# peterropac/Aegolius

Measured on AMD Instinct MI355X. Metric: Mpoints/sec SDF eval, 1024^3 grid, 10-prim smooth-union tree, higher is better.
Workload: dtype f32

## Files before the change

### aegolius_amd/_engine.py

```python
import atexit
import contextlib
import ctypes
import importlib.util
import os
import sys
import threading

import numpy as np

_HERE = os.path.dirname(os.path.abspath(__file__))
LIB_PATH = os.path.join(_HERE, "libsdfk.so")

MODE_AUTO, MODE_INTERPRET, MODE_SPECIALIZED, MODE_NOCULL = 0, 1, 2, 3
(FLAVOUR_PLAIN_ARRAY, FLAVOUR_PLAIN_GRID, FLAVOUR_TILE_ARRAY, FLAVOUR_TILE_GRID, FLAVOUR_TILE_MASK, FLAVOUR_ROWS_ARRAY,
 FLAVOUR_ROWS_GRID, FLAVOUR_ROWS_MASK, FLAVOUR_ROWS2D_ARRAY, FLAVOUR_ROWS2D_GRID, FLAVOUR_RAYS, FLAVOUR_OCCUPANCY) = range(12)
FLAVOUR_FLAGS = 0x100
FLAVOUR_XY = 0x200

_c = ctypes
_vp, _i64, _int, _sz = _c.c_void_p, _c.c_int64, _c.c_int, _c.c_size_t
_fp = _c.POINTER(_c.c_float)

SIGNATURES = {
    "sdfk_abi_version": (_int, []),
    "sdfk_device_count": (_int, []),
    "sdfk_last_error": (_c.c_char_p, []),
    "sdfk_program_create": (_vp, [_vp, _sz, _vp, _sz, _vp, _sz, _int]),
    "sdfk_program_destroy": (None, [_vp]),
    "sdfk_program_set_params": (_int, [_vp, _vp, _sz]),
    "sdfk_program_set_cull": (_int, [_vp, _vp, _sz, _vp]),
    "sdfk_program_source": (_c.c_char_p, [_vp]),
    "sdfk_program_compile_check": (_int, [_vp, _c.POINTER(_sz)]),
    "sdfk_program_chain_members": (_int, [_vp]),
    "sdfk_program_compile_flavour": (_int, [_vp, _int, _c.POINTER(_sz), _c.POINTER(_c.c_double)]),
    "sdfk_debug_compile_external": (_int, [_vp, _int, _c.POINTER(_sz)]),
    "sdfk_debug_jit_stats": (None, [_c.POINTER(_i64), _c.POINTER(_c.c_double)]),
    "sdfk_jit_drain": (None, []),
    "sdfk_jit_cancel": (None, []),
    "sdfk_debug_set_rtc_defs": (None, [_c.c_char_p]),
    "sdfk_eval_device": (_int, [_vp, _vp, _i64, _i64, _vp, _vp, _int]),
    "sdfk_eval_device_rows": (_int, [_vp, _vp, _i64, _i64, _i64, _vp, _vp, _int]),
    "sdfk_eval_device_rows2d": (_int, [_vp, _vp, _i64, _i64, _i64, _vp, _vp, _int]),
    "sdfk_eval_device_rows2d_xy": (_int, [_vp, _vp, _i64, _i64, _i64, _vp, _vp, _int]),
    "sdfk_debug_cells_stats": (None, [_int, _c.POINTER(_c.c_longlong)]),
    "sdfk_debug_rays_stats": (None, [_int, _c.POINTER(_c.c_longlong)]),
    "sdfk_eval_device_rows3d": (_int, [_vp, _vp, _i64, _i64, _i64, _i64, _i64, _vp, _vp, _int]),
    "sdfk_debug_row_masks": (_int, [_vp, _vp, _i64, _i64, _i64, _vp, _c.POINTER(_i64), _c.POINTER(_int), _vp]),
    "sdfk_eval_grid_sharded": (_int, [_vp, _vp, _i64, _vp, _i64, _vp, _i64, _int, _vp, _vp, _int]),
    "sdfk_eval_grid_sharded_device": (_int, [_vp, _vp, _i64, _vp, _i64, _vp, _i64, _int, _vp, _int, _vp, _int]),
    "sdfk_eval_device_aux": (_int, [_vp, _vp, _i64, _i64, _vp, _int, _i64, _vp, _vp, _int]),
    "sdfk_eval_grid_aux": (_int, [_vp, _vp, _i64, _vp, _i64, _vp, _i64, _i64, _i64, _vp, _int, _i64, _vp, _vp, _int]),
    "sdfk_field_min": (_int, [_vp, _i64, _c.POINTER(_c.c_float), _vp]),
    "sdfk_grid_box_average": (_int, [_vp, _i64, _i64, _i64, _int, _int, _int, _int, _vp, _vp]),
    "sdfk_grid_edge_detect": (_int, [_vp, _i64, _i64, _i64, _vp, _vp]),
# ... 114 lines not shown
        with _lock:
            if _lib is None:
                if not os.path.exists(LIB_PATH):
                    raise SdfkError(
                        "aegolius_amd: %s is missing - build it with "
                        "`python -c 'import __graft_entry__ as g; g.build()'` (needs hipcc, gfx950). "
                        "There is no CPU path." % LIB_PATH)
                _share_torch_hip_runtime()
                handle = ctypes.CDLL(LIB_PATH)
                for name, (res, args) in SIGNATURES.items():
                    fn = getattr(handle, name)
                    fn.restype, fn.argtypes = res, args
                if handle.sdfk_abi_version() != 1:
                    raise SdfkError("libsdfk.so ABI version mismatch")
                atexit.register(handle.sdfk_jit_cancel)
                _lib = handle
    return _lib


def last_error():
    msg = lib().sdfk_last_error()
    return msg.decode("utf-8", "replace") if msg else ""


def check(rc, what):
    if rc != 0:
        raise SdfkError("%s failed (%d): %s" % (what, rc, last_error()))


def device_count():
# ... 581 lines not shown
```

### aegolius_amd/csrc/sdfk.hip

```cpp
#include <hip/hip_runtime.h>
#include <hip/hiprtc.h>

#include <chrono>
#include <algorithm>
#include <atomic>
#include <cmath>
#include <condition_variable>
#include <cstdio>
#include <cstdlib>
#include <cstring>
#include <deque>
#include <functional>
#include <map>
#include <memory>
#include <mutex>
#include <thread>
#include <string>
#include <vector>
#include <dirent.h>
#include <dlfcn.h>
#include <fcntl.h>
#include <signal.h>
#include <spawn.h>
#include <sys/wait.h>
// ... 1053 lines not shown
    if (e->state == 0) {
        e->state = 1;
        lk.unlock();
        const std::string src = make_source();
        if (wait || !rtc_helper_available()) {
            code_build(e, src, rwb);
        } else {
            g_builds.post([e, src, rwb] { code_build(e, src, rwb, true); });
        }
        return e;
    }
    if (wait) e->cv.wait(lk, [&] { return e->state != 1; });
    return e;
}
static std::string flavour_key(const sdfk_program* p, int flavour, int rwb, int with_flags = 0) {
    return p->key + "|f" + std::to_string(flavour) + ((with_flags & 1) ? "s" : "") + ((with_flags & 2) ? "x" : "") + "|" + rtc_option_key(rwb);
}
static std::string flavour_source(const sdfk_program* p, int flavour, int with_flags = 0) {
    return std::string((with_flags & 1) ? "#define SDFK_FLAGS 1\n" : "") + ((with_flags & 2) ? "#define SDFK_XY 1\n" : "") +
           sdfk_generate_source(g_ops, SDFK_OP_COUNT, p->code.data(), p->code.size() / 2, p->result_reg, p->sites, flavour,
                                &p->sites_all);
}

extern "C" int sdfk_program_chain_members(const sdfk_program* p) {
    return p && p->chain_mode ? p->chain_members : 0;
}
extern "C" int sdfk_program_compile_check(sdfk_program* p, size_t* code_size) {
    if (!p) return fail(-1, "null program");
    size_t total = 0;
    const int rwb = rows_geo(p);
    for (int f = 0; f < SDFK_FL_COUNT; ++f) {
        if (f == SDFK_FL_RAYS) continue;
        if (f == SDFK_FL_OCCUPANCY) continue;
        if (p->sites.empty() && f != SDFK_FL_PLAIN_ARRAY && f != SDFK_FL_PLAIN_GRID) continue;
// ... 310 lines not shown
            g_cells_stats[6] = (long long)all; g_cells_stats[7] = (long long)empty;
        }
        if (trace) fprintf(stderr, "[sdfk cells] %d members: fine %ux%ux%u = %llu cells (2^%u planes x 2^%u blocks x 2^%u windows), coarse %llu; pool %u of %llu entries; "
                "fine lists: mean %.1f max %llu, %llu without a list, %llu empty\n", p->chain_members, fine.ncx, fine.ncy, fine.ncz, nf, fine.lx, fine.ly, fine.lz, nc,
                head, cap, (double)sum / (double)std::max<unsigned long long>(1, nf - all - empty), mx, all, empty);
    }
    out->lv = fine;
    out->sph = b + o_fsph;
    out->span = b + o_fspan;
    out->cand = b + o_pool;
    out->enabled = 1u;
    out->ncells = (unsigned)nf;
    return 0;
}

static int run(sdfk_program* p, const SrcArray* arr, const SrcGrid* grid, long long n, float* d_out, void* stream_,
               int mode, bool vec_ok, long long row_len = 0, const float* aux = nullptr, long long aux_stride = 0,
               bool flat = false, long long plane_rows = 0, long long plane_phase = 0, unsigned* d_flags = nullptr,
               unsigned thr_key = 0, bool xy = false) {
    if (!p) return fail(-1, "null program");
    if (n < 0) return fail(-1, "negative point count");
    if (p->n_aux > 0 && (!aux || aux_stride < n))
        return fail(-1, "this program reads auxiliary fields (staged evaluation): use sdfk_eval_device_aux / sdfk_eval_grid_aux");
    if (n == 0) return 0;
    if (mode == SDFK_MODE_AUTO) mode = g_default_mode;
    if (d_flags && (mode == SDFK_MODE_AUTO || mode == SDFK_MODE_INTERPRET)) mode = SDFK_MODE_SPECIALIZED;
    if (xy) {
        if (!arr || p->n_aux > 0) return fail(-1, "two-row coordinates: array source, no auxiliary fields");
        if (mode == SDFK_MODE_AUTO || mode == SDFK_MODE_INTERPRET) mode = SDFK_MODE_SPECIALIZED;
    }
    hipStream_t stream = (hipStream_t)stream_;
    int device = 0;
    HIPCHK(hipGetDevice(&device));
    DevState* d = nullptr;
// ... 23 lines not shown
        if (arr && rows_geometry(n, row_len, &rg, (flat || d_flags) ? 0 : plane_rows, plane_phase, p->chain_mode))
            flavour = (flat || xy) ? SDFK_FL_ROWS2D_ARRAY : SDFK_FL_ROWS_ARRAY;
        else if (arr && vec_ok && !p->chain_mode && !d_flags && !xy) flavour = SDFK_FL_TILE_ARRAY;
        else if (grid && grid->start % grow == 0 &&
                 rows_geometry(n, grow, &rg, (grid->n2 > 1 && !d_flags) ? (long long)grid->n1 : 0,
                               grid->n2 > 1 ? (grid->start / grow) % (long long)grid->n1 : 0, p->chain_mode))
            flavour = grid->n2 > 1 ? SDFK_FL_ROWS_GRID : SDFK_FL_ROWS2D_GRID;
        else if (grid && vec_ok && !p->chain_mode && !d_flags) flavour = SDFK_FL_TILE_GRID;
        if (!p->chain_mode && (long long)(p->code.size() / 2) > rows_limit &&
            (flavour == SDFK_FL_ROWS_ARRAY || flavour == SDFK_FL_ROWS2D_ARRAY || flavour == SDFK_FL_ROWS_GRID || flavour == SDFK_FL_ROWS2D_GRID)) {
            const bool is_arr = arr != nullptr;
            if (vec_ok && !d_flags && !xy) flavour = is_arr ? SDFK_FL_TILE_ARRAY : SDFK_FL_TILE_GRID;
            else if (!d_flags) flavour = is_arr ? SDFK_FL_PLAIN_ARRAY : SDFK_FL_PLAIN_GRID;
        }
    }
    std::shared_ptr<SpecModule> sk;
    if (mode != SDFK_MODE_INTERPRET) {
        static const bool async_jit = [] { const char* e = getenv("SDFK_ASYNC_JIT"); return !(e && e[0] == '0'); }();
        const bool wait = mode != SDFK_MODE_AUTO || !p->interp_ok || !async_jit;
        std::string err;
        sk = get_module(p, device, flavour, wait, &err, (d_flags ? 1 : 0) | (xy ? 2 : 0));
        if (sk && sk->failed) {
            if (mode == SDFK_MODE_SPECIALIZED || !p->interp_ok)
                return fail(-3, "specialised kernel unavailable: " + err);
            static bool warned = false;
            if (!warned) {
                fprintf(stderr, "[sdfk] hiprtc specialisation failed, using the interpreter kernel: %s\n", err.c_str());
                warned = true;
            }
            sk.reset();
        }
    }
    if (!sk && !p->interp_ok)
        return fail(-4, "program needs more registers than the interpreter kernel has (use the specialised mode)");

    const float* prm = d->d_params;
// ... 13 lines not shown
                    void* src[] = {&co, &stride};
                    rc = prepare_cells(p, d, sk->fn[1], rg, src, 2, prm, tab, stream, &cells);
                    if (rc) return rc;
                }
                void* args[] = {&prm, &tab, &co, &stride, &rg, &d_out, &d_flags, &thr_key, &cells};
                HIPCHK(hipModuleLaunchKernel(sk->fn[0], tiles, 1, 1, rthreads, 1, 1, 0, stream, args, nullptr));
            } else {
                SrcGrid g = *grid;
                rg.row0 = grid->start / grow;
                rg.yrows = grid->n2 > 1 ? 0 : 1;
                if (with_cells) {
                    void* src[] = {&g};
                    rc = prepare_cells(p, d, sk->fn[1], rg, src, 1, prm, tab, stream, &cells);
                    if (rc) return rc;
                }
                void* args[] = {&prm, &tab, &g, &rg, &d_out, &d_flags, &thr_key, &cells};
                HIPCHK(hipModuleLaunchKernel(sk->fn[0], tiles, 1, 1, rthreads, 1, 1, 0, stream, args, nullptr));
            }
            return 0;
        }
        if (flavour == SDFK_FL_TILE_ARRAY || flavour == SDFK_FL_TILE_GRID) {
            const unsigned tiles = (unsigned)((n + tile_points() - 1) / tile_points());
            if (arr) {
                const float* co = arr->co;
                long long stride = arr->stride;
                void* args[] = {&prm, &tab, &co, &stride, &n, &d_out};
                HIPCHK(hipModuleLaunchKernel(sk->fn[0], tiles, 1, 1, tile_threads(), 1, 1, 0, stream, args, nullptr));
            } else {
                SrcGrid g = *grid;
                void* args[] = {&prm, &tab, &g, &n, &d_out};
                HIPCHK(hipModuleLaunchKernel(sk->fn[0], tiles, 1, 1, tile_threads(), 1, 1, 0, stream, args, nullptr));
// ... 188 lines not shown
    if (n == 1) {
        out[0] = (float)lo;
        return 0;
    }
    const double div = (double)(n - 1);
    const double delta = hi - lo;
    const double step = delta / div;
    for (int64_t i = 0; i < n; ++i) {
        volatile double t = (step != 0.0) ? (double)i * step : ((double)i / div) * delta;
        out[i] = (float)(t + lo);
    }
    out[n - 1] = (float)hi;
    return 0;
}

struct AxisTables {
    float* d = nullptr;
    ~AxisTables() {
        if (d) (void)hipFree(d);
    }
};

static int upload_axes(const float* ax0, int64_t n0, const float* ax1, int64_t n1, const float* ax2, int64_t n2,
                       hipStream_t stream, AxisTables* t, SrcGrid* g, int64_t start) {
    if (!ax0 || !ax1 || !ax2 || n0 < 1 || n1 < 1 || n2 < 1) return fail(-1, "grid axes missing or empty");
    if (n1 > 0x7fffffff || n2 > 0x7fffffff) return fail(-1, "grid axis too long");
    HIPCHK(hipMalloc(&t->d, (size_t)(n0 + n1 + n2) * sizeof(float)));
    HIPCHK(hipMemcpyAsync(t->d, ax0, (size_t)n0 * sizeof(float), hipMemcpyHostToDevice, stream));
    HIPCHK(hipMemcpyAsync(t->d + n0, ax1, (size_t)n1 * sizeof(float), hipMemcpyHostToDevice, stream));
    HIPCHK(hipMemcpyAsync(t->d + n0 + n1, ax2, (size_t)n2 * sizeof(float), hipMemcpyHostToDevice, stream));
    g->ax0 = t->d;
    g->ax1 = t->d + n0;
    g->ax2 = t->d + n0 + n1;
    g->n1 = (unsigned)n1;
    g->n2 = (unsigned)n2;
    g->start = start;
    return 0;
}

extern "C" int sdfk_eval_grid(sdfk_program* p, const float* ax0, int64_t n0, const float* ax1, int64_t n1,
                              const float* ax2, int64_t n2, int64_t start, int64_t count, float* d_out, void* stream,
                              int mode) {
    if (!d_out) return fail(-1, "sdfk_eval_grid: null output");
    if (start < 0 || count < 0 || start + count > n0 * n1 * n2) return fail(-1, "sdfk_eval_grid: range outside the grid");
    AxisTables t;
    SrcGrid g;
    int rc = upload_axes(ax0, n0, ax1, n1, ax2, n2, (hipStream_t)stream, &t, &g, start);
    if (rc) return rc;
    rc = run(p, nullptr, &g, count, d_out, stream, mode, aligned16(d_out));
    if (rc) return rc;
    HIPCHK(hipStreamSynchronize((hipStream_t)stream));
    return 0;
}

extern "C" int sdfk_eval_grid_aux(sdfk_program* p, const float* ax0, int64_t n0, const float* ax1, int64_t n1,
                                  const float* ax2, int64_t n2, int64_t start, int64_t count, const float* d_aux, int n_aux,
                                  int64_t aux_stride, float* d_out, void* stream, int mode) {
    if (!p || !d_out) return fail(-1, "sdfk_eval_grid_aux: null pointer");
    if (start < 0 || count < 0 || start + count > n0 * n1 * n2) return fail(-1, "sdfk_eval_grid_aux: range outside the grid");
    if (n_aux < p->n_aux) return fail(-1, "sdfk_eval_grid_aux: the program reads more auxiliary fields than were passed");
    AxisTables t;
    SrcGrid g;
    int rc = upload_axes(ax0, n0, ax1, n1, ax2, n2, (hipStream_t)stream, &t, &g, start);
    if (rc) return rc;
    rc = run(p, nullptr, &g, count, d_out, stream, mode, aligned16(d_out), 0, d_aux, aux_stride);
    if (rc) return rc;
    HIPCHK(hipStreamSynchronize((hipStream_t)stream));
    return 0;
}

extern "C" int sdfk_eval_grid_host(sdfk_program* p, const float* ax0, int64_t n0, const float* ax1, int64_t n1,
                                   const float* ax2, int64_t n2, int64_t start, int64_t count, float* out, int device,
                                   int mode) {
    if (!p) return fail(-1, "null program");
    if (count < 0 || (count > 0 && !out)) return fail(-1, "sdfk_eval_grid_host: bad arguments");
    if (start < 0 || start + count > n0 * n1 * n2) return fail(-1, "sdfk_eval_grid_host: range outside the grid");
    if (count == 0) return 0;
    HIPCHK(hipSetDevice(device));
    int64_t chunk = std::min<int64_t>(count, (int64_t)1 << 27);
    const int64_t grow = n2 > 1 ? n2 : n1;
    if (start % grow == 0 && chunk > grow) chunk = chunk / grow * grow;
    float* d_out = nullptr;
    HIPCHK(hipMalloc(&d_out, (size_t)chunk * sizeof(float)));
    AxisTables t;
    SrcGrid g;
    int rc = upload_axes(ax0, n0, ax1, n1, ax2, n2, nullptr, &t, &g, start);
    for (int64_t s = 0; s < count && rc == 0; s += chunk) {
        const int64_t m = std::min(chunk, count - s);
        g.start = start + s;
        rc = run(p, nullptr, &g, m, d_out, nullptr, mode, true);
        if (rc == 0 && hipMemcpy(out + s, d_out, (size_t)m * sizeof(float), hipMemcpyDeviceToHost) != hipSuccess)
            rc = fail(-6, "sdfk_eval_grid_host: device-to-host copy failed");
    }
    (void)hipFree(d_out);
    return rc;
}

extern "C" int sdfk_eval_grid_sharded(sdfk_program* p, const float* ax0, int64_t n0, const float* ax1, int64_t n1,
                                      const float* ax2, int64_t n2, int n_shards, const int* devices, float* out,
                                      int mode) {
    if (!p || !out) return fail(-1, "sdfk_eval_grid_sharded: null argument");
    if (n_shards < 1 || n_shards > 64) return fail(-1, "sdfk_eval_grid_sharded: 1..64 shards");
    if (!ax0 || !ax1 || !ax2 || n0 < 1 || n1 < 1 || n2 < 1) return fail(-1, "grid axes missing or empty");
    int n_dev = 0;
    if (hipGetDeviceCount(&n_dev) != hipSuccess || n_dev < 1) return fail(-8, "sdfk_eval_grid_sharded: no HIP device");
// ... 367 lines not shown
```

### aegolius_amd/csrc/sdfk_codegen.cpp

```cpp
#include "sdfk_codegen.h"

#include <algorithm>
#include <cstdio>
#include <cstring>
#include <map>
#include <set>

#include "sdfk_embedded.inc"

std::string sdfk_vector_prelude() { return std::string(kEmbeddedDevice) + "\n" + kEmbeddedVecdev + "\n"; }

static const char kWrappers[] = R"SDFKW(
template <int VEC, typename SRC>
static __device__ __forceinline__ void sdfk_body(const float* __restrict__ PRM, const float* __restrict__ TAB,
                                                 const SRC& src, long long off, long long n,
                                                 float* __restrict__ out, const float* __restrict__ aux,
                                                 long long aux_stride, unsigned* __restrict__ flags, unsigned thr) {
    const long long block_base = (long long)sdfk_bx() * (SDFK_BLOCK * VEC);
    const unsigned lane_off = sdfk_tx() * VEC;
#ifdef SDFK_FLAGS                                              // the flag-writing build of this flavour (its own code object:
    {                                                          // carried as a run-time branch it cost the field kernels registers)
        const bool active = block_base + lane_off < n;
        unsigned nib = 0u;
        if (active) {
// ... 1678 lines not shown
static const char kRowsGrid[] = R"SDFKR(
// the same on a regular grid expanded from three per-axis tables (no coordinate array: 4 B/point); the slab
// starts at a row boundary and out[0] is its first point
extern "C" __global__ __launch_bounds__(64 * SDFK_RWAVES) void sdfk_spec_rg(
    const float* __restrict__ PRM, const float* __restrict__ TAB, SrcGrid s, sdfk_rowgeom g, float* __restrict__ out,
    unsigned* __restrict__ flags, unsigned thr SDFK_CELLS_KARG) {
    sdfk_rows_kernel(PRM, TAB, s, g, out, flags, thr SDFK_CELLS_PASS);
}
#ifdef SDFK_CELLS
extern "C" __global__ __launch_bounds__(256) void sdfk_spec_cellsg(
    const float* __restrict__ PRM, const float* __restrict__ TAB, SrcGrid s, sdfk_rowgeom g, sdfk_cellpass cp) {
    sdfk_cells_kernel(PRM, TAB, s, g, cp);
}
#endif
)SDFKR";
static const char kRowsMask[] = R"SDFKR(
// test aid: the skip masks (two 64-bit words per brick: sites 0-31, 32-63; bit 2k = first operand of site k
// skipped, bit 2k+1 = second) followed by the "uniform rows" flag in a third word
extern "C" __global__ __launch_bounds__(64 * SDFK_RWAVES) void sdfk_spec_rmask(
    const float* __restrict__ PRM, const float* __restrict__ TAB, const float* __restrict__ co, long long stride,
    sdfk_rowgeom g, unsigned long long* __restrict__ masks) {
    __shared__ __attribute__((aligned(16))) sdfk_rowmeta meta;
    const SrcArray s = {co, stride};
    unsigned rb, c;
    sdfk_rows_prepare(PRM, TAB, s, g, &meta, sdfk_bx(), rb, c);
    const unsigned q = sdfk_bx() * SDFK_RNBRICK + sdfk_tx();
    if (sdfk_tx() < SDFK_RNBRICK && q < g.nbricks) {
        masks[3ull * q] = meta.mask[0][sdfk_tx()];
        masks[3ull * q + 1] = meta.mask[1][sdfk_tx()];
        masks[3ull * q + 2] = meta.uniform[sdfk_tx()];
// ... 980 lines not shown
               "    return x;\n}\n";
        g.simt = g.analyse_leaves();
        if (g.simt) {
            char def[160];
            snprintf(def, sizeof def, "\n#ifndef SDFK_NOSIMT\n#define SDFK_SIMT 1\n#endif\n#define SDFK_NLEAF %zu\n", g.leaves.size());
            g.s += def;
            g.s += kSimtGeometry;
            g.emit_groups();
            g.emit_probe_leaves();
            g.emit_probe_fold();
        }
        g.emit_probe();
        g.emit_rows_culled(result_reg);
        g.s += kRowsKernel;
        if (all || flavour == SDFK_FL_ROWS_ARRAY || flavour == SDFK_FL_ROWS2D_ARRAY) g.s += kRowsArray;
        if (all || flavour == SDFK_FL_ROWS_GRID || flavour == SDFK_FL_ROWS2D_GRID) g.s += kRowsGrid;
        if (all || flavour == SDFK_FL_ROWS_MASK) g.s += kRowsMask;
    }
    return g.s;
}
```

### aegolius_amd/csrc/sdfk_occupancy.inc

```
#include "sdfk_occdev.h"

template <int NC, int NV, typename SRC>
__global__ __launch_bounds__(SDFK_OCC_BLOCK) void sdfk_occ_interp_kernel(const uint2* __restrict__ code, int n_instr,
                                                                        const float* __restrict__ prm,
                                                                        const float* __restrict__ tab, int result_reg, SRC src,
                                                                        sdfk_occgrid grid, float* __restrict__ out) {
    const SdfkInterpField<NC, NV> field = {code, n_instr, prm, tab, result_reg};
    sdfk_occ_sample(src, field, grid, out);
}

#define SDFK_OCC_RUN 1024
#define SDFK_OCC_PARTIALS 4096

struct sdfk_occclass {
    const float* __restrict__ ax0;
    const float* __restrict__ ax1;
    const float* __restrict__ ax2;
    const float* __restrict__ hw0;
    const float* __restrict__ hw1;
    const float* __restrict__ hw2;
    unsigned n1, n2;
    long long first, count;
    float level, lip;
    unsigned level_key;
// ... 173 lines not shown
    const unsigned k0 = n0 > 1 ? samples : 1, k1 = n1 > 1 ? samples : 1, k2 = n2 > 1 ? samples : 1;
    auto lg = [](unsigned k) { return k == 8 ? 3u : k == 4 ? 2u : k == 2 ? 1u : 0u; };
    const unsigned K = k0 * k1 * k2;
    const int64_t total_cells = n0 * n1 * n2;
    const int64_t slab = occ_slab_cells(n0, n1, n2, slab_cells);

    hipStream_t stream = (hipStream_t)stream_;
    int device = 0;
    HIPCHK(hipGetDevice(&device));
    DevState* d = nullptr;
    int rc = ensure_resident(p, device, stream, &d);
    if (rc) return rc;

    AxisTables axes, extra;
    SrcGrid g;
    rc = upload_axes(ax0, n0, ax1, n1, ax2, n2, stream, &axes, &g, 0);
    if (rc) return rc;
    const size_t s0 = (size_t)n0 * k0, s1 = (size_t)n1 * k1, s2 = (size_t)n2 * k2;
    HIPCHK(hipMalloc(&extra.d, (s0 + s1 + s2 + (size_t)(n0 + n1 + n2)) * sizeof(float)));
    float* d_sub[3] = {extra.d, extra.d + s0, extra.d + s0 + s1};
    float* d_hw[3] = {extra.d + s0 + s1 + s2, extra.d + s0 + s1 + s2 + n0, extra.d + s0 + s1 + s2 + n0 + n1};
    HIPCHK(hipMemcpyAsync(d_sub[0], sub0, s0 * sizeof(float), hipMemcpyHostToDevice, stream));
    HIPCHK(hipMemcpyAsync(d_sub[1], sub1, s1 * sizeof(float), hipMemcpyHostToDevice, stream));
    HIPCHK(hipMemcpyAsync(d_sub[2], sub2, s2 * sizeof(float), hipMemcpyHostToDevice, stream));
    HIPCHK(hipMemcpyAsync(d_hw[0], hw0, (size_t)n0 * sizeof(float), hipMemcpyHostToDevice, stream));
    HIPCHK(hipMemcpyAsync(d_hw[1], hw1, (size_t)n1 * sizeof(float), hipMemcpyHostToDevice, stream));
    HIPCHK(hipMemcpyAsync(d_hw[2], hw2, (size_t)n2 * sizeof(float), hipMemcpyHostToDevice, stream));

    char* scratch = (char*)d_scratch;
    unsigned long long* d_partial = (unsigned long long*)scratch;
    unsigned long long* d_blk = (unsigned long long*)(scratch + SDFK_OCC_PARTIALS * 8);
// ... 11 lines not shown
    sdfk_occclass C = {g.ax0, g.ax1, g.ax2, d_hw[0], d_hw[1], d_hw[2], (unsigned)n1, (unsigned)n2, 0, 0, level, lipschitz,
                       sdfk_sel_key(level)};
    const float* prm = d->d_params;
    const float* tab = d->d_tables;
    const int n_instr = (int)(p->code.size() / 2);
    const unsigned per_wave = K >= 64u ? 1u : 64u / K;
    int64_t near_total = 0;

    for (int64_t first = 0; first < total_cells; first += slab) {
        const int64_t cells = std::min(slab, total_cells - first);
        float* out = d_fraction + first;
        unsigned long long n_entries = (unsigned long long)cells;
        if (pass_ms) HIPCHK(hipEventRecord(ev.e[0], stream));
        if (skip) {
            g.start = first;
            rc = run(p, nullptr, &g, cells, d_centre, stream, mode, true);
            if (rc) return rc;
            if (pass_ms) HIPCHK(hipEventRecord(ev.e[1], stream));
            C.first = first;
            C.count = cells;
            const long long runs = occ_runs(cells);
            const unsigned blocks = (unsigned)((runs + SDFK_OCC_BLOCK / 64 - 1) / (SDFK_OCC_BLOCK / 64));
            hipLaunchKernelGGL(sdfk_occ_classify_kernel<false>, dim3(blocks), dim3(SDFK_OCC_BLOCK), 0, stream,
                               (const float*)d_centre, C, out, d_list, d_blk);
            hipLaunchKernelGGL(sdfk_select_scan_kernel, dim3(1), dim3(1024), 0, stream, d_blk, runs);
            hipLaunchKernelGGL(sdfk_occ_classify_kernel<true>, dim3(blocks), dim3(SDFK_OCC_BLOCK), 0, stream,
                               (const float*)d_centre, C, out, d_list, d_blk);
            HIPCHK(hipGetLastError());
            unsigned long long h = 0;
            HIPCHK(hipMemcpyAsync(&h, d_blk + runs, sizeof h, hipMemcpyDeviceToHost, stream));
            HIPCHK(hipStreamSynchronize(stream));
// ... 69 lines not shown
```

### include/sdfk.h

```cpp
#ifndef SDFK_H
#define SDFK_H

#include <stddef.h>
#include <stdint.h>

#ifdef __cplusplus
extern "C" {
#endif

#define SDFK_ABI_VERSION 1

#define SDFK_MODE_AUTO 0
#define SDFK_MODE_INTERPRET 1
#define SDFK_MODE_SPECIALIZED 2
#define SDFK_MODE_NOCULL 3

typedef struct sdfk_program sdfk_program;

int sdfk_abi_version(void);
int sdfk_device_count(void);
const char* sdfk_last_error(void);

sdfk_program* sdfk_program_create(const uint32_t* code, size_t n_instr, const float* params, size_t n_params,
                                  const float* tables, size_t n_tables, int result_reg);
// ... 13 lines not shown
#define SDFK_FLAVOUR_ROWS_MASK 7
#define SDFK_FLAVOUR_ROWS2D_ARRAY 8
#define SDFK_FLAVOUR_ROWS2D_GRID 9
#define SDFK_FLAVOUR_RAYS 10
#define SDFK_FLAVOUR_OCCUPANCY 11
#define SDFK_FLAVOUR_FLAGS 0x100
#define SDFK_FLAVOUR_XY 0x200
int sdfk_program_compile_flavour(sdfk_program* prog, int flavour, size_t* code_size, double* seconds);
void sdfk_debug_cells_stats(int enable, long long* out8);
void sdfk_debug_rays_stats(int enable, long long* out8);
int sdfk_debug_compile_external(sdfk_program* prog, int flavour, size_t* code_size);
void sdfk_jit_drain(void);
void sdfk_jit_cancel(void);
void sdfk_debug_jit_stats(int64_t* builds, double* seconds);
void sdfk_debug_set_rtc_defs(const char* defs);

int sdfk_eval_device(sdfk_program* prog, const float* d_co, int64_t n, int64_t row_stride, float* d_out,
                     void* stream, int mode);
int sdfk_eval_device_rows(sdfk_program* prog, const float* d_co, int64_t n, int64_t row_stride, int64_t row_len,
                          float* d_out, void* stream, int mode);
int sdfk_eval_device_rows3d(sdfk_program* prog, const float* d_co, int64_t n, int64_t row_stride, int64_t row_len,
                            int64_t plane_rows, int64_t first_row_in_plane, float* d_out, void* stream, int mode);
int sdfk_eval_device_rows2d(sdfk_program* prog, const float* d_co, int64_t n, int64_t row_stride, int64_t row_len,
                            float* d_out, void* stream, int mode);
int sdfk_eval_device_rows2d_xy(sdfk_program* prog, const float* d_xy, int64_t n, int64_t row_stride, int64_t row_len,
                               float* d_out, void* stream, int mode);
int sdfk_eval_host(sdfk_program* prog, const void* co, int co_dtype, int64_t n, int64_t row_stride, float* out,
                   int device, int mode);
int sdfk_eval_host_resident(sdfk_program* prog, const void* co, int co_dtype, int64_t n, int64_t row_stride,
                            float* d_out, int device, int mode);
// ... 161 lines not shown
```

Measured before the change: 365,500.

## Add lean rows-grid kernel with analytic brick bounds and cached axis tables

Adds a new rows-grid kernel variant that derives each brick's bounding sphere directly from the first and last axis-table entries when the axes are monotone, rather than computing bounds from loaded coordinates. It also splits sub-bricks at plane boundaries for tighter culling and uses a precomputed reciprocal to divide row indices. Axis tables are now cached on the device across calls (up to 8 entries, keyed by content), which avoids a malloc and host-to-device upload each call. The cache compares full axis contents on every call, holds device memory until exit, and falls back to the legacy kernel when the axes are not monotone or index ranges overflow.

```diff
diff --git a/aegolius_amd/_engine.py b/aegolius_amd/_engine.py
--- a/aegolius_amd/_engine.py
+++ b/aegolius_amd/_engine.py
@@ -38,6 +38,8 @@
     "sdfk_jit_drain": (None, []),
     "sdfk_jit_cancel": (None, []),
     "sdfk_debug_set_rtc_defs": (None, [_c.c_char_p]),
+    "sdfk_debug_axis_monotone": (_int, [_vp, _i64]),
+    "sdfk_axes_cache_clear": (None, []),
     "sdfk_eval_device": (_int, [_vp, _vp, _i64, _i64, _vp, _vp, _int]),
     "sdfk_eval_device_rows": (_int, [_vp, _vp, _i64, _i64, _i64, _vp, _vp, _int]),
     "sdfk_eval_device_rows2d": (_int, [_vp, _vp, _i64, _i64, _i64, _vp, _vp, _int]),
@@ -182,6 +184,7 @@
                 if handle.sdfk_abi_version() != 1:
                     raise SdfkError("libsdfk.so ABI version mismatch")
                 atexit.register(handle.sdfk_jit_cancel)
+                atexit.register(handle.sdfk_axes_cache_clear)
                 _lib = handle
     return _lib
 
diff --git a/aegolius_amd/csrc/sdfk.hip b/aegolius_amd/csrc/sdfk.hip
--- a/aegolius_amd/csrc/sdfk.hip
+++ b/aegolius_amd/csrc/sdfk.hip
@@ -1091,10 +1091,12 @@
     return e;
 }
 static std::string flavour_key(const sdfk_program* p, int flavour, int rwb, int with_flags = 0) {
-    return p->key + "|f" + std::to_string(flavour) + ((with_flags & 1) ? "s" : "") + ((with_flags & 2) ? "x" : "") + "|" + rtc_option_key(rwb);
+    return p->key + "|f" + std::to_string(flavour) + ((with_flags & 1) ? "s" : "") + ((with_flags & 2) ? "x" : "") +
+           ((with_flags & 4) ? "g" : "") + "|" + rtc_option_key(rwb);
 }
 static std::string flavour_source(const sdfk_program* p, int flavour, int with_flags = 0) {
     return std::string((with_flags & 1) ? "#define SDFK_FLAGS 1\n" : "") + ((with_flags & 2) ? "#define SDFK_XY 1\n" : "") +
+           ((with_flags & 4) ? "#define SDFK_GRID_LEGACY 1\n" : "") +
            sdfk_generate_source(g_ops, SDFK_OP_COUNT, p->code.data(), p->code.size() / 2, p->result_reg, p->sites, flavour,
                                 &p->sites_all);
 }
@@ -1435,10 +1437,13 @@
     return 0;
 }
 
+struct GridInfo {
+    bool lean_ok = false;
+};
 static int run(sdfk_program* p, const SrcArray* arr, const SrcGrid* grid, long long n, float* d_out, void* stream_,
                int mode, bool vec_ok, long long row_len = 0, const float* aux = nullptr, long long aux_stride = 0,
                bool flat = false, long long plane_rows = 0, long long plane_phase = 0, unsigned* d_flags = nullptr,
-               unsigned thr_key = 0, bool xy = false) {
+               unsigned thr_key = 0, bool xy = false, const GridInfo* gi = nullptr) {
     if (!p) return fail(-1, "null program");
     if (n < 0) return fail(-1, "negative point count");
     if (p->n_aux > 0 && (!aux || aux_stride < n))
@@ -1492,12 +1497,15 @@
             else if (!d_flags) flavour = is_arr ? SDFK_FL_PLAIN_ARRAY : SDFK_FL_PLAIN_GRID;
         }
     }
+    const bool grid_rows = grid && (flavour == SDFK_FL_ROWS_GRID || flavour == SDFK_FL_ROWS2D_GRID);
+    const bool grid_legacy = grid_rows && !p->chain_mode && !d_flags &&
+                             !(gi && gi->lean_ok && grow <= (1LL << 30) && grid->start / grow + rg.R < (1LL << 32));
     std::shared_ptr<SpecModule> sk;
     if (mode != SDFK_MODE_INTERPRET) {
         static const bool async_jit = [] { const char* e = getenv("SDFK_ASYNC_JIT"); return !(e && e[0] == '0'); }();
         const bool wait = mode != SDFK_MODE_AUTO || !p->interp_ok || !async_jit;
         std::string err;
-        sk = get_module(p, device, flavour, wait, &err, (d_flags ? 1 : 0) | (xy ? 2 : 0));
+        sk = get_module(p, device, flavour, wait, &err, (d_flags ? 1 : 0) | (xy ? 2 : 0) | (grid_legacy ? 4 : 0));
         if (sk && sk->failed) {
             if (mode == SDFK_MODE_SPECIALIZED || !p->interp_ok)
                 return fail(-3, "specialised kernel unavailable: " + err);
@@ -1541,7 +1549,8 @@
                     rc = prepare_cells(p, d, sk->fn[1], rg, src, 1, prm, tab, stream, &cells);
                     if (rc) return rc;
                 }
-                void* args[] = {&prm, &tab, &g, &rg, &d_out, &d_flags, &thr_key, &cells};
+                unsigned inv_n1 = (unsigned)std::min<unsigned long long>(0xffffffffull, (1ull << 32) / (unsigned long long)g.n1);
+                void* args[] = {&prm, &tab, &g, &rg, &d_out, &d_flags, &thr_key, with_cells ? (void*)&cells : (void*)&inv_n1};
                 HIPCHK(hipModuleLaunchKernel(sk->fn[0], tiles, 1, 1, rthreads, 1, 1, 0, stream, args, nullptr));
             }
             return 0;
@@ -1760,7 +1769,39 @@
     return 0;
 }
 
+extern "C" int sdfk_debug_axis_monotone(const float* a, int64_t n) {
+    if (!a || n < 1) return 0;
+    int m = 3;
+    for (int64_t i = 0; i < n; ++i) {
+        unsigned bits;
+        memcpy(&bits, &a[i], sizeof bits);
+        if ((bits & 0x7f800000u) == 0x7f800000u) return 0;
+        if (i > 0 && a[i] < a[i - 1]) m &= ~1;
+        if (i > 0 && a[i] > a[i - 1]) m &= ~2;
+    }
+    return m;
+}
+
+struct AxisEntry {
+    int device = 0;
+    std::vector<float> host;
+    int64_t n0 = 0, n1 = 0, n2 = 0;
+    float* d = nullptr;
+    int mono[3] = {0, 0, 0};
+    ~AxisEntry() {
+        if (d) (void)hipFree(d);
+    }
+};
+static std::mutex g_axes_mu;
+static std::vector<std::shared_ptr<AxisEntry>>& g_axes = *new std::vector<std::shared_ptr<AxisEntry>>();
+static const size_t kAxesCached = 8;
+extern "C" void sdfk_axes_cache_clear(void) {
+    std::lock_guard<std::mutex> lk(g_axes_mu);
+    g_axes.clear();
+}
+
 struct AxisTables {
+    std::shared_ptr<AxisEntry> e;
     float* d = nullptr;
     ~AxisTables() {
         if (d) (void)hipFree(d);
@@ -1768,19 +1809,51 @@
 };
 
 static int upload_axes(const float* ax0, int64_t n0, const float* ax1, int64_t n1, const float* ax2, int64_t n2,
-                       hipStream_t stream, AxisTables* t, SrcGrid* g, int64_t start) {
+                       hipStream_t stream, AxisTables* t, SrcGrid* g, int64_t start, GridInfo* gi = nullptr) {
     if (!ax0 || !ax1 || !ax2 || n0 < 1 || n1 < 1 || n2 < 1) return fail(-1, "grid axes missing or empty");
     if (n1 > 0x7fffffff || n2 > 0x7fffffff) return fail(-1, "grid axis too long");
-    HIPCHK(hipMalloc(&t->d, (size_t)(n0 + n1 + n2) * sizeof(float)));
-    HIPCHK(hipMemcpyAsync(t->d, ax0, (size_t)n0 * sizeof(float), hipMemcpyHostToDevice, stream));
-    HIPCHK(hipMemcpyAsync(t->d + n0, ax1, (size_t)n1 * sizeof(float), hipMemcpyHostToDevice, stream));
-    HIPCHK(hipMemcpyAsync(t->d + n0 + n1, ax2, (size_t)n2 * sizeof(float), hipMemcpyHostToDevice, stream));
-    g->ax0 = t->d;
-    g->ax1 = t->d + n0;
-    g->ax2 = t->d + n0 + n1;
+    int device = 0;
+    HIPCHK(hipGetDevice(&device));
+    const size_t b0 = (size_t)n0 * sizeof(float), b1 = (size_t)n1 * sizeof(float), b2 = (size_t)n2 * sizeof(float);
+    {
+        std::lock_guard<std::mutex> lk(g_axes_mu);
+        for (size_t i = 0; i < g_axes.size() && !t->e; ++i) {
+            const std::shared_ptr<AxisEntry>& c = g_axes[i];
+            if (c->device == device && c->n0 == n0 && c->n1 == n1 && c->n2 == n2 && memcmp(c->host.data(), ax0, b0) == 0 &&
+                memcmp(c->host.data() + n0, ax1, b1) == 0 && memcmp(c->host.data() + n0 + n1, ax2, b2) == 0) {
+                t->e = c;
+                std::rotate(g_axes.begin(), g_axes.begin() + (std::ptrdiff_t)i, g_axes.begin() + (std::ptrdiff_t)i + 1);
+            }
+        }
+        if (!t->e) {
+            std::shared_ptr<AxisEntry> c = std::make_shared<AxisEntry>();
+            c->device = device;
+            c->n0 = n0;
+            c->n1 = n1;
+            c->n2 = n2;
+            c->host.resize((size_t)(n0 + n1 + n2));
+            memcpy(c->host.data(), ax0, b0);
+            memcpy(c->host.data() + n0, ax1, b1);
+            memcpy(c->host.data() + n0 + n1, ax2, b2);
+            c->mono[0] = sdfk_debug_axis_monotone(ax0, n0);
+            c->mono[1] = sdfk_debug_axis_monotone(ax1, n1);
+            c->mono[2] = sdfk_debug_axis_monotone(ax2, n2);
+            HIPCHK(hipMalloc(&c->d, c->host.size() * sizeof(float)));
+            HIPCHK(hipMemcpyAsync(c->d, c->host.data(), c->host.size() * sizeof(float), hipMemcpyHostToDevice, stream));
+            HIPCHK(hipStreamSynchronize(stream));
+            g_axes.insert(g_axes.begin(), c);
+            if (g_axes.size() > kAxesCached) g_axes.pop_back();
+            t->e = c;
+        }
+    }
+    const AxisEntry& e = *t->e;
+    g->ax0 = e.d;
+    g->ax1 = e.d + n0;
+    g->ax2 = e.d + n0 + n1;
     g->n1 = (unsigned)n1;
     g->n2 = (unsigned)n2;
     g->start = start;
+    if (gi) gi->lean_ok = e.mono[0] && e.mono[1] && e.mono[2] && (n2 > 1 || e.host[(size_t)(n0 + n1)] == 0.0f);
     return 0;
 }
 
@@ -1791,9 +1864,10 @@
     if (start < 0 || count < 0 || start + count > n0 * n1 * n2) return fail(-1, "sdfk_eval_grid: range outside the grid");
     AxisTables t;
     SrcGrid g;
-    int rc = upload_axes(ax0, n0, ax1, n1, ax2, n2, (hipStream_t)stream, &t, &g, start);
+    GridInfo gi;
+    int rc = upload_axes(ax0, n0, ax1, n1, ax2, n2, (hipStream_t)stream, &t, &g, start, &gi);
     if (rc) return rc;
-    rc = run(p, nullptr, &g, count, d_out, stream, mode, aligned16(d_out));
+    rc = run(p, nullptr, &g, count, d_out, stream, mode, aligned16(d_out), 0, nullptr, 0, false, 0, 0, nullptr, 0, false, &gi);
     if (rc) return rc;
     HIPCHK(hipStreamSynchronize((hipStream_t)stream));
     return 0;
@@ -1807,9 +1881,10 @@
     if (n_aux < p->n_aux) return fail(-1, "sdfk_eval_grid_aux: the program reads more auxiliary fields than were passed");
     AxisTables t;
     SrcGrid g;
-    int rc = upload_axes(ax0, n0, ax1, n1, ax2, n2, (hipStream_t)stream, &t, &g, start);
+    GridInfo gi;
+    int rc = upload_axes(ax0, n0, ax1, n1, ax2, n2, (hipStream_t)stream, &t, &g, start, &gi);
     if (rc) return rc;
-    rc = run(p, nullptr, &g, count, d_out, stream, mode, aligned16(d_out), 0, d_aux, aux_stride);
+    rc = run(p, nullptr, &g, count, d_out, stream, mode, aligned16(d_out), 0, d_aux, aux_stride, false, 0, 0, nullptr, 0, false, &gi);
     if (rc) return rc;
     HIPCHK(hipStreamSynchronize((hipStream_t)stream));
     return 0;
@@ -1830,11 +1905,12 @@
     HIPCHK(hipMalloc(&d_out, (size_t)chunk * sizeof(float)));
     AxisTables t;
     SrcGrid g;
-    int rc = upload_axes(ax0, n0, ax1, n1, ax2, n2, nullptr, &t, &g, start);
+    GridInfo gi;
+    int rc = upload_axes(ax0, n0, ax1, n1, ax2, n2, nullptr, &t, &g, start, &gi);
     for (int64_t s = 0; s < count && rc == 0; s += chunk) {
         const int64_t m = std::min(chunk, count - s);
         g.start = start + s;
-        rc = run(p, nullptr, &g, m, d_out, nullptr, mode, true);
+        rc = run(p, nullptr, &g, m, d_out, nullptr, mode, true, 0, nullptr, 0, false, 0, 0, nullptr, 0, false, &gi);
         if (rc == 0 && hipMemcpy(out + s, d_out, (size_t)m * sizeof(float), hipMemcpyDeviceToHost) != hipSuccess)
             rc = fail(-6, "sdfk_eval_grid_host: device-to-host copy failed");
     }
diff --git a/aegolius_amd/csrc/sdfk_codegen.cpp b/aegolius_amd/csrc/sdfk_codegen.cpp
--- a/aegolius_amd/csrc/sdfk_codegen.cpp
+++ b/aegolius_amd/csrc/sdfk_codegen.cpp
@@ -1716,6 +1716,304 @@
 }
 #endif
 )SDFKR";
+static const char kRowsGridLean[] = R"SDFKR(
+#if !defined(SDFK_GRID_LEGACY) && !defined(SDFK_FLAGS) && !defined(SDFK_CHAIN)
+#define SDFK_GRID_LEAN 1
+struct sdfk_leanmeta {
+    uint4 brick[SDFK_RNBRICK];                  // x: plane of the brick's first row (SDFK_FLAT: its global row), y: its index in the
+                                                // plane, z: window, w: live rows | ((first local row * L) mod 32) << 8; w = 0: no brick
+    unsigned long long mask[SDFK_NMASK][SDFK_RNBRICK];
+#ifdef SDFK_SIMT
+    float4 cen[SDFK_NCEN];
+    float leafval[SDFK_NLEAF * SDFK_NCEN];
+#endif
+};
+// brick (row block rb, window c), wave-uniform; inv_n1 = floor(2^32 / n1)
+static __device__ __forceinline__ uint4 sdfk_lean_brick(const SrcGrid& s, const sdfk_rowgeom& g, unsigned inv_n1, unsigned rb,
+                                                        unsigned c, long long& r0) {
+    long long rend;
+    sdfk_block_rows(g, rb, r0, rend);
+    unsigned nrows = 0u;
+    if (r0 < rend) nrows = rend - r0 < SDFK_RROWS ? (unsigned)(rend - r0) : (unsigned)SDFK_RROWS;
+    const unsigned g0 = (unsigned)(g.row0 + r0);
+#ifdef SDFK_FLAT
+    const unsigned ix = g0, iy = 0u;
+    (void)inv_n1;
+#else
+    const unsigned ix = sdfk_udiv(g0, s.n1, inv_n1), iy = g0 - ix * s.n1;
+#endif
+    return make_uint4(ix, iy, c, nrows | ((((unsigned)r0 * g.L) & 31u) << 8));
+}
+// point index (in its row) of the first point of the brick's window in row r of the brick: windows are aligned in the
+// flat array, so they shift from row to row unless L is a multiple of 32
+static __device__ __forceinline__ int sdfk_lean_win(const sdfk_rowgeom& g, uint4 d, int r) {
+    return 32 * (int)d.z - (int)(((d.w >> 8) + (unsigned)r * (g.L & 31u)) & 31u);
+}
+#if defined(SDFK_SIMT) && SDFK_NSUB == 8 && !defined(SDFK_FLAT)
+// Two row parts per brick: a brick whose rows come from two planes is split where the plane changes instead of in the
+// middle (as sdfk_sub_centre does), so that each part lies in one plane and is bounded tightly. Rows of the first part.
+static __device__ __forceinline__ int sdfk_lean_split(const SrcGrid& s, uint4 d) {
+    const unsigned nrows = d.w & 0xffu, sp = s.n1 - d.y;
+    return (sp < nrows && nrows - sp <= s.n1) ? (int)sp : SDFK_RROWS / 2;
+}
+#endif
+// Bounding sphere of rows [ra, rb) x points [i0, i0 + np) of the windows of a live brick: the box between the first and
+// last table entries touched — over ALL of its rows: the windows shift —, centre = its midpoint, radius = its half
+// diagonal with the inflation of sdfk_rows_bounds. Points outside the row count as the row's nearest point, rows past
+// the block's last one as that one (as in sdfk_rows_load: they are never stored).
+static __device__ __forceinline__ float4 sdfk_lean_sphere(const SrcGrid& s, const sdfk_rowgeom& g, uint4 d, int ra, int rb,
+                                                          int i0, int np) {
+    const int nrows = (int)(d.w & 0xffu), last = (int)g.L - 1;
+    rb = rb < nrows ? rb : nrows;
+    ra = ra < rb - 1 ? ra : rb - 1;
+    // smallest and largest shift of the window over the rows (sdfk_lean_win, row after row)
+    const unsigned step = g.L & 31u;
+    unsigned sh = ((d.w >> 8) + (unsigned)ra * step) & 31u, shmin = 31u, shmax = 0u;
+#pragma unroll 1
+    for (int r = ra; r < rb; ++r) {
+        shmin = sh < shmin ? sh : shmin;
+        shmax = sh > shmax ? sh : shmax;
+        sh = (sh + step) & 31u;
+    }
+    const int zlo = min(max(32 * (int)d.z + i0 - (int)shmax, 0), last);
+    const int zhi = min(max(32 * (int)d.z + i0 - (int)shmin + np - 1, 0), last);
+#ifdef SDFK_FLAT
+    // (x, y, z) = (ax0[row], ax1[point], ax2[0])
+    const float xa = s.ax0[d.x + (unsigned)ra], xb = s.ax0[d.x + (unsigned)(rb - 1)];
+    const float ta = s.ax1[zlo], tb = s.ax1[zhi];
+    const float cx = 0.5f * (xa + xb), ct = 0.5f * (ta + tb);
+    const float hx = sd_rawmax(sd_abs(xa - cx), sd_abs(xb - cx)), ht = sd_rawmax(sd_abs(ta - ct), sd_abs(tb - ct));
+    return make_float4(cx, ct, s.ax2[0], 1.00001f * sqrtf(sd_fma(ht, ht, hx * hx)) + 1e-30f);
+#else
+    unsigned ixa = d.x, iya = d.y + (unsigned)ra, ixb = d.x, iyb = d.y + (unsigned)(rb - 1);
+    while (iya >= s.n1) { iya -= s.n1; ++ixa; }
+    while (iyb >= s.n1) { iyb -= s.n1; ++ixb; }
+    if (ixa != ixb) { iya = 0u; iyb = s.n1 - 1u; }               // rows of more than one plane: the whole second axis
+    const float xa = s.ax0[ixa], xb = s.ax0[ixb], ya = s.ax1[iya], yb = s.ax1[iyb], ta = s.ax2[zlo], tb = s.ax2[zhi];
+    const float cx = 0.5f * (xa + xb), cy = 0.5f * (ya + yb), ct = 0.5f * (ta + tb);
+    const float hx = sd_rawmax(sd_abs(xa - cx), sd_abs(xb - cx)), hy = sd_rawmax(sd_abs(ya - cy), sd_abs(yb - cy));
+    const float ht = sd_rawmax(sd_abs(ta - ct), sd_abs(tb - ct));
+    return make_float4(cx, cy, ct, 1.00001f * sqrtf(sd_fma(ht, ht, sd_fma(hx, hx, hy * hy))) + 1e-30f);
+#endif
+}
+// the sphere sub-brick sb of a live brick is culled with (one sub-brick: the whole brick)
+static __device__ __forceinline__ float4 sdfk_lean_centre(const SrcGrid& s, const sdfk_rowgeom& g, uint4 d, unsigned sb) {
+#if defined(SDFK_SIMT) && SDFK_NSUB > 1
+    constexpr int NZP = 4, NRP = SDFK_NSUB / NZP, RPS = SDFK_RROWS / NRP, ZPS = SDFK_RZ / NZP;
+    int ra = (int)(sb / NZP) * RPS, rb = ra + RPS;
+#if SDFK_NSUB == 8 && !defined(SDFK_FLAT)
+    const int sp = sdfk_lean_split(s, d);
+    ra = sb / NZP ? sp : 0;
+    rb = sb / NZP ? SDFK_RROWS : sp;
+#endif
+    return sdfk_lean_sphere(s, g, d, ra, rb, (int)(sb % NZP) * ZPS, ZPS);
+#else
+    (void)sb;
+    return sdfk_lean_sphere(s, g, d, 0, SDFK_RROWS, 0, SDFK_RZ);
+#endif
+}
+#ifdef SDFK_DEBUG_GRID_BOUNDS
+// the sub-brick of row lr, points [zq, zq + 8) of the window (test aid below)
+static __device__ __forceinline__ unsigned sdfk_lean_sub_of(const SrcGrid& s, uint4 d, int lr, int zq) {
+#if defined(SDFK_SIMT) && SDFK_NSUB > 1
+    constexpr int NZP = 4, NRP = SDFK_NSUB / NZP, RPS = SDFK_RROWS / NRP, ZPS = SDFK_RZ / NZP;
+    static_assert(ZPS == 2 * SDFK_NP, "a lane's points lie in one sub-brick");
+    int part = lr / RPS;
+#if SDFK_NSUB == 8 && !defined(SDFK_FLAT)
+    part = lr >= sdfk_lean_split(s, d) ? 1 : 0;
+#endif
+    return (unsigned)(part * NZP + zq / ZPS);
+#else
+    return 0u;
+#endif
+}
+#endif
+
+static __device__ __forceinline__ void sdfk_rows_kernel_lean(const float* __restrict__ PRM, const float* __restrict__ TAB,
+                                                             const SrcGrid& s, const sdfk_rowgeom& g, unsigned inv_n1,
+                                                             float* __restrict__ out) {
+    __shared__ __attribute__((aligned(16))) sdfk_leanmeta meta;
+    const int lane = sdfk_tx() & 63, wave = __builtin_amdgcn_readfirstlane(sdfk_tx() >> 6);
+    const int lr = lane / SDFK_RLPR;
+    const int zq = (lane % SDFK_RLPR) * (2 * SDFK_NP);
+#pragma unroll 1
+  for (unsigned tt = 0; tt < SDFK_RTILES; ++tt) {
+    // (the tile order of sdfk_rows_kernel: runs of SDFK_XGROUP tiles per XCD)
+    const unsigned xg_t = sdfk_bx() / 8;
+    const unsigned tile = (((xg_t / SDFK_XGROUP) * 8 + sdfk_bx() % 8) * SDFK_XGROUP + xg_t % SDFK_XGROUP) * SDFK_RTILES + tt;
+    if (tile * SDFK_RNBRICK >= g.nbricks) break;
+    if (tt) __syncthreads();
+    const unsigned q0 = tile * SDFK_RNBRICK + wave * SDFK_RWBRICKS;            // first brick of this wave
+    const unsigned rb0 = sdfk_udiv(q0, g.nchunk, g.inv_nchunk), c0 = q0 - rb0 * g.nchunk;
+    // phase A, what is left of it: one descriptor per brick
+    {
+        unsigned rb = rb0, c = c0;
+#pragma unroll
+        for (int j = 0; j < SDFK_RWBRICKS; ++j) {
+            long long r0;
+            uint4 d = sdfk_lean_brick(s, g, inv_n1, rb, c, r0);
+            if (q0 + j >= g.nbricks) d.w = 0u;                     // (the launch is padded with bricks beyond the last one)
+            if (lane == 0) {
+                meta.brick[wave * SDFK_RWBRICKS + j] = d;
+#ifdef SDFK_SIMT
+#pragma unroll
+                for (int w = 0; w < SDFK_NMASK; ++w) meta.mask[w][wave * SDFK_RWBRICKS + j] = ~0ull;   // the fold lanes AND their decisions into these
+#endif
+            }
+            if (++c == g.nchunk) { c = 0; ++rb; }
+        }
+    }
+    __syncthreads();
+    // phase B: the probe of sdfk_rows_prepare, centres from the tables
+#ifdef SDFK_SIMT
+    if (sdfk_tx() < SDFK_NCEN) {
+        const uint4 d = meta.brick[sdfk_tx() / SDFK_NSUB];
+        float4 cc = make_float4(0.0f, 0.0f, 0.0f, 1.0f);           // a dead brick still meets a probe lane: harmless values
+#ifndef SDFK_ABLATE_BOUNDS
+        if (d.w & 0xffu) cc = sdfk_lean_centre(s, g, d, sdfk_tx() % SDFK_NSUB);
+#endif
+        meta.cen[sdfk_tx()] = cc;
+    }
+    __syncthreads();
+#ifndef SDFK_ABLATE_PROBE
+    sdfk_probe_leaves(meta.cen, meta.leafval, PRM, TAB);
+    __syncthreads();
+    if (sdfk_tx() < SDFK_NCEN && tile * SDFK_RNBRICK + sdfk_tx() / SDFK_NSUB < g.nbricks) {
+        const float4 cc = meta.cen[sdfk_tx()];
+        V3T<float> ctr = {cc.x, cc.y, cc.z};
+        unsigned long long mk[SDFK_NMASK];
+        sdfk_probe_fold(meta.leafval, sdfk_tx(), ctr, cc.w, PRM, mk);
+#pragma unroll
+        for (int w = 0; w < SDFK_NMASK; ++w)
+            __hip_atomic_fetch_and(&meta.mask[w][sdfk_tx() / SDFK_NSUB], mk[w], __ATOMIC_RELAXED, __HIP_MEMORY_SCOPE_WORKGROUP);
+    }
+#endif
+#else
+    if (sdfk_tx() < SDFK_RNBRICK && tile * SDFK_RNBRICK + sdfk_tx() < g.nbricks) {
+        const uint4 d = meta.brick[sdfk_tx()];
+        float4 bb = make_float4(0.0f, 0.0f, 0.0f, 1.0f);
+#ifndef SDFK_ABLATE_BOUNDS
+        if (d.w & 0xffu) bb = sdfk_lean_centre(s, g, d, 0u);
+#endif
+        V3T<float> ctr = {bb.x, bb.y, bb.z};
+        unsigned long long mk[SDFK_NMASK];
+#pragma unroll
+        for (int w = 0; w < SDFK_NMASK; ++w) mk[w] = 0ull;
+#ifndef SDFK_ABLATE_PROBE
+        sdfk_probe_r(ctr, bb.w, PRM, TAB, mk);
+#endif
+#pragma unroll
+        for (int w = 0; w < SDFK_NMASK; ++w) meta.mask[w][sdfk_tx()] = mk[w];
+    }
+#endif
+    __syncthreads();
+    // phase C: a lane owns 2 * SDFK_NP consecutive points of one row
+    unsigned rb = rb0, c = c0;
+#pragma unroll 1
+    for (int j = 0; j < SDFK_RWBRICKS; ++j) {
+        if (q0 + j >= g.nbricks) break;
+        const int b = wave * SDFK_RWBRICKS + j;
+        const unsigned k = c;
+        long long r0;
+        const uint4 d = sdfk_lean_brick(s, g, inv_n1, rb, k, r0);
+        if (++c == g.nchunk) { c = 0; ++rb; }
+        const int nrows = (int)(d.w & 0xffu);
+        if (nrows == 0) continue;
+        unsigned mw[2 * SDFK_NMASK];                             // the brick's skip bits as scalar words
+#pragma unroll
+        for (int w = 0; w < SDFK_NMASK; ++w) {
+            const unsigned long long m = meta.mask[w][b];
+            mw[2 * w] = __builtin_amdgcn_readfirstlane((unsigned)m);
+            mw[2 * w + 1] = __builtin_amdgcn_readfirstlane((unsigned)(m >> 32));
+        }
+        const bool interior = sdfk_interior(g.L, k);
+        const bool live_row = lr < nrows;
+        const int dr = live_row ? lr : nrows - 1;
+        const int z = sdfk_lean_win(g, d, dr) + zq;              // this lane's first point in its row (edge windows: may lie outside)
+        const int last = (int)g.L - 1;
+        // the row's coordinates and the lane's entries of the table along the row
+#ifdef SDFK_FLAT
+        const float X = s.ax0[d.x + (unsigned)dr], Y = s.ax2[0]; // (x, z): the host has checked that z is 0
+        const float* __restrict__ along = s.ax1;
+#else
+        unsigned ix = d.x, iy = d.y + (unsigned)dr;
+        while (iy >= s.n1) { iy -= s.n1; ++ix; }
+        const float X = s.ax0[ix], Y = s.ax1[iy];
+        const float* __restrict__ along = s.ax2;
+#endif
+        f2 T[SDFK_NP];
+        if (interior) {
+#pragma unroll
+            for (int q = 0; q < SDFK_NP; q += 2) {
+                const sdfk_f4u v = *reinterpret_cast<const sdfk_f4u*>(along + z + 2 * q);
+                T[q] = {v.x, v.y};
+                T[q + 1] = {v.z, v.w};
+            }
+        } else {
+            SDFK_EACH T[q] = {along[min(max(z + 2 * q, 0), last)], along[min(max(z + 2 * q + 1, 0), last)]};
+        }
+        V3P P[SDFK_NP];
+        f2 res[SDFK_NP];
+#ifdef SDFK_FLAT
+        SDFK_EACH { P[q].x = sp<f2>(X); P[q].y = T[q]; P[q].z = sp<f2>(Y); }
+#else
+        SDFK_EACH { P[q].x = sp<f2>(X); P[q].y = sp<f2>(Y); P[q].z = T[q]; }
+#endif
+#ifdef SDFK_ABLATE_EVAL
+        SDFK_EACH res[q] = T[q] + __builtin_bit_cast(float, mw[0] ^ mw[1] ^ mw[2] ^ mw[3]);
+#else
+        sdfk_rows_culled<true>(X, Y, P, mw, PRM, TAB, res);
+#endif
+#ifdef SDFK_DEBUG_GRID_BOUNDS
+        {   // test aid: instead of the field, 0 where the point lies inside the sphere its (sub-)brick was culled with, else 1
+            const float4 cc = sdfk_lean_centre(s, g, d, sdfk_lean_sub_of(s, d, dr, zq));
+            SDFK_EACH {
+                const f2 ex = P[q].x - cc.x, ey = P[q].y - cc.y, ez = P[q].z - cc.z;
+                const f2 e2 = sd_fma(ez, ez, sd_fma(ex, ex, ey * ey));
+                res[q] = {sqrtf(e2.x) <= cc.w ? 0.0f : 1.0f, sqrtf(e2.y) <= cc.w ? 0.0f : 1.0f};
+            }
+        }
+#endif
+        if (live_row) {
+            float* po = out + (r0 * (long long)g.L + (long long)((unsigned long long)(unsigned)dr * g.L) + z);
+            if (interior) {
+#pragma unroll
+                for (int q = 0; q < SDFK_NP; q += 2) {
+                    sdfk_f4u v = {res[q].x, res[q].y, res[q + 1].x, res[q + 1].y};
+                    __builtin_nontemporal_store(v, reinterpret_cast<sdfk_f4u*>(po + 2 * q));
+                }
+            } else {
+                // an edge window: a quad that lies wholly inside the row is still one store (nothing is loaded here whose
+                // round trips a per-lane branch could serialise); at most one quad per row end straddles it and goes point
+                // by point. -DSDFK_LEAN_EDGE_POINTS: every point on its own, as in sdfk_rows_kernel.
+#pragma unroll
+                for (int q = 0; q < SDFK_NP; q += 2) {
+#ifndef SDFK_LEAN_EDGE_POINTS
+                    if (z + 2 * q >= 0 && z + 2 * q + 3 <= last) {
+                        sdfk_f4u v = {res[q].x, res[q].y, res[q + 1].x, res[q + 1].y};
+                        __builtin_nontemporal_store(v, reinterpret_cast<sdfk_f4u*>(po + 2 * q));
+                        continue;
+                    }
+#endif
+                    if (z + 2 * q >= 0 && z + 2 * q <= last) po[2 * q] = res[q].x;
+                    if (z + 2 * q + 1 >= 0 && z + 2 * q + 1 <= last) po[2 * q + 1] = res[q].y;
+                    if (z + 2 * q + 2 >= 0 && z + 2 * q + 2 <= last) po[2 * q + 2] = res[q + 1].x;
+                    if (z + 2 * q + 3 >= 0 && z + 2 * q + 3 <= last) po[2 * q + 3] = res[q + 1].y;
+                }
+            }
+        }
+    }
+  }
+}
+extern "C" __global__ __launch_bounds__(64 * SDFK_RWAVES) void sdfk_spec_rg(
+    const float* __restrict__ PRM, const float* __restrict__ TAB, SrcGrid s, sdfk_rowgeom g, float* __restrict__ out,
+    unsigned* __restrict__ flags, unsigned thr, unsigned inv_n1) {
+    (void)flags;
+    (void)thr;
+    sdfk_rows_kernel_lean(PRM, TAB, s, g, inv_n1, out);
+}
+#else
+)SDFKR";
 static const char kRowsMask[] = R"SDFKR(
 // test aid: the skip masks (two 64-bit words per brick: sites 0-31, 32-63; bit 2k = first operand of site k
 // skipped, bit 2k+1 = second) followed by the "uniform rows" flag in a third word
@@ -2726,7 +3024,11 @@
         g.emit_rows_culled(result_reg);
         g.s += kRowsKernel;
         if (all || flavour == SDFK_FL_ROWS_ARRAY || flavour == SDFK_FL_ROWS2D_ARRAY) g.s += kRowsArray;
-        if (all || flavour == SDFK_FL_ROWS_GRID || flavour == SDFK_FL_ROWS2D_GRID) g.s += kRowsGrid;
+        if (all || flavour == SDFK_FL_ROWS_GRID || flavour == SDFK_FL_ROWS2D_GRID) {
+            g.s += kRowsGridLean;
+            g.s += kRowsGrid;
+            g.s += "#endif\n";
+        }
         if (all || flavour == SDFK_FL_ROWS_MASK) g.s += kRowsMask;
     }
     return g.s;
diff --git a/aegolius_amd/csrc/sdfk_occupancy.inc b/aegolius_amd/csrc/sdfk_occupancy.inc
--- a/aegolius_amd/csrc/sdfk_occupancy.inc
+++ b/aegolius_amd/csrc/sdfk_occupancy.inc
@@ -211,7 +211,8 @@
 
     AxisTables axes, extra;
     SrcGrid g;
-    rc = upload_axes(ax0, n0, ax1, n1, ax2, n2, stream, &axes, &g, 0);
+    GridInfo gi;
+    rc = upload_axes(ax0, n0, ax1, n1, ax2, n2, stream, &axes, &g, 0, &gi);
     if (rc) return rc;
     const size_t s0 = (size_t)n0 * k0, s1 = (size_t)n1 * k1, s2 = (size_t)n2 * k2;
     HIPCHK(hipMalloc(&extra.d, (s0 + s1 + s2 + (size_t)(n0 + n1 + n2)) * sizeof(float)));
@@ -253,7 +254,7 @@
         if (pass_ms) HIPCHK(hipEventRecord(ev.e[0], stream));
         if (skip) {
             g.start = first;
-            rc = run(p, nullptr, &g, cells, d_centre, stream, mode, true);
+            rc = run(p, nullptr, &g, cells, d_centre, stream, mode, true, 0, nullptr, 0, false, 0, 0, nullptr, 0, false, &gi);
             if (rc) return rc;
             if (pass_ms) HIPCHK(hipEventRecord(ev.e[1], stream));
             C.first = first;
diff --git a/include/sdfk.h b/include/sdfk.h
--- a/include/sdfk.h
+++ b/include/sdfk.h
@@ -51,6 +51,8 @@
 void sdfk_jit_cancel(void);
 void sdfk_debug_jit_stats(int64_t* builds, double* seconds);
 void sdfk_debug_set_rtc_defs(const char* defs);
+int sdfk_debug_axis_monotone(const float* table, int64_t n);
+void sdfk_axes_cache_clear(void);
 
 int sdfk_eval_device(sdfk_program* prog, const float* d_co, int64_t n, int64_t row_stride, float* d_out,
                      void* stream, int mode);
```

Result: no change. 364,900 (-0.2%).
